# JADGardner/neusky

Hardware: AMD Instinct MI355X
Metric: train rays/sec on NeRF-OSR lk2 @1024 rays x 96 samples (higher is better)
Workload: dtype f32 in memory; forward products: fp16 hi + residual split, 3 x v_mfma_f32_32x32x16_f16 per product on power-of-two pre-scaled operands, one fp32 accumulator (~2^-22): FiLM-SIREN chains and the SDF / albedo field alike; backward products: the same fp16 split on per-row / per-matrix pre-scaled gradien; 1 GPU; full NeuSky train step (BASELINE configs[2]): 1024 rays/GPU x 96 samples, proposal 256+96, 512 illumination directions (256 upper-hemisphere DDF queries/ray), illumination decoder = this project's FiLM-SIREN H = 128 (RENI-shaped: latent 100x3; the reference's configured Attention decoder is absent from its tree), hash L16 F2 T2^19 x2, 256-wide MLPs; fwd + losses + bwd + all-reduce + 5 Adam groups; rays_per_gpu=1024, samples_per_ray=96, illumination_directions=512, parallelism=ray-sharded dp1, launcher=self-spawned, launch=HIP graph replay (1 graph/step + all-reduce + 5 Adam launches)

## Files before the change

neusky_amd/csrc/film_chain.hip:

```cpp
#include "chain.h"

namespace {

constexpr int FWD_FRAG_BUFFERS = 3;


struct Layout {
  int NT, Gc, Gx, Gh;
  long base_map, base_film0, base_film, base_head, total_groups;
  int n_tiles;
};

__host__ __device__ inline Layout fwd_layout(const nsky_film_net& n) {
  Layout L;
  L.NT = n.hidden / 32;
  L.Gc = groups_of(n.cond_dim);
  L.Gx = groups_of(n.x_dim);
  L.Gh = groups_of(n.hidden);
  L.base_map = (long)L.NT * L.Gc;
  L.base_film0 = L.base_map + (long)(n.n_map - 1) * L.NT * L.Gh;
  L.base_film = L.base_film0 + (long)L.NT * (2 * L.Gh + L.Gx);
  L.base_head = L.base_film + (long)(n.n_film - 1) * L.NT * 3 * L.Gh;
  L.total_groups = L.base_head + L.Gh;
  L.n_tiles = n.n_map * L.NT + n.n_film * L.NT * 3 + 1;
// ... 128 lines not shown

struct FwdArgs {
  nsky_film_net net;
  const unsigned char* stream;
  const float* table;
  const float* cond; int ldcond;
  const float* x; int ldx;
  int M;
  float* h_save[MAXL];
  float* z_save[MAXL];
  float* y_save[MAXL];
  float* res; int ldres;
};


template <int H, int KSC>
__global__ __launch_bounds__(256, 1) void film_fwd_kernel(const FwdArgs a) {
  constexpr int NT = H / 32, KS = H / 16;
  __shared__ __attribute__((aligned(16))) unsigned char smem[RING_BYTES + (BIAS_FLOATS + SCALE_FLOATS) * 4];
  float* bl = reinterpret_cast<float*>(smem + RING_BYTES);
  const nsky_film_net& net = a.net;
  const int tid = threadIdx.x, lane = tid & 63;
  const int wave = __builtin_amdgcn_readfirstlane(tid >> 6);
  const int c = lane & 31, h = lane >> 5;
  float* sl = bl + BIAS_FLOATS;
  {
    constexpr int N4 = (BIAS_FLOATS + SCALE_FLOATS) / 4;
    float4 q[(N4 + 255) / 256];
#pragma unroll
    for (int i = 0; i < (N4 + 255) / 256; ++i)
      if (i * 256 + tid < N4) q[i] = ldg4(a.table + 4 * (i * 256 + tid));
// ... 94 lines not shown
  }
  f16x8 xh[1], xl[1];
  const float x_inv = load_planes<1>(a.x + rowc * a.ldx, (net.x_dim + 3) & ~3, 1, h, xh, xl);
  f16x8 yh[KS], yl[KS];
#pragma unroll
  for (int ks = 0; ks < KS; ++ks)
#pragma unroll
    for (int j = 0; j < 8; ++j) { yh[ks][j] = (_Float16)0.0f; yl[ks][j] = (_Float16)0.0f; }
  const float* bias_mo = bl + n_map * H;
  const float* bias_film = bias_mo + 2 * n_film * H;
  for (int i = 0; i < n_film; ++i) {
    const float* bF = bias_mo + i * H;
    const float* bP = bias_mo + (n_film + i) * H;
    const float* bZ = bias_film + i * H;
    float* zblk = a.z_save[i] ? a.z_save[i] + (wave_live ? rt : 0) * NT * 1024 : nullptr;
    float* yblk = a.y_save[i] + (wave_live ? rt : 0) * NT * 1024;
    for (int t = 0; t < NT; ++t) {
      f32x16 aF, aP, aZ;
#pragma unroll
      for (int r = 0; r < 16; ++r) { aF[r] = 0.0f; aP[r] = 0.0f; aZ[r] = 0.0f; }
      product<KS, 4, false, RING_GROUPS, FWD_FRAG_BUFFERS>(ws, hh, hl, aF);
      product<KS, 4, false, RING_GROUPS, FWD_FRAG_BUFFERS>(ws, hh, hl, aP);
      float z_unscale;
      if (i == 0) {
        product<1>(ws, xh, xl, aZ);
        z_unscale = x_inv;
      } else {
        product<KS, 4, false, RING_GROUPS, FWD_FRAG_BUFFERS>(ws, yh, yl, aZ);
        z_unscale = 1.0f / Y_SCALE;
      }
      const float iF = h_inv * sl[tile], iP = h_inv * sl[tile + 1], iZ = z_unscale * sl[tile + 2];
// ... 4 lines not shown
        const int fo = 32 * t + 8 * g + 4 * h;
        const float4 b4F = *reinterpret_cast<const float4*>(bF + fo);
        const float4 b4P = *reinterpret_cast<const float4*>(bP + fo);
        const float4 b4Z = *reinterpret_cast<const float4*>(bZ + fo);
        const float bf[4] = {b4F.x, b4F.y, b4F.z, b4F.w}, bp[4] = {b4P.x, b4P.y, b4P.z, b4P.w}, bz[4] = {b4Z.x, b4Z.y, b4Z.z, b4Z.w};
#pragma unroll
        for (int q = 0; q < 4; ++q) {
          const int r = 4 * g + q;
          const float F = fmaf(aF[r], iF, bf[q]), P = fmaf(aP[r], iP, bp[q]), z = fmaf(aZ[r], iZ, bz[q]);
          zz[r] = z;
          yy[r] = sin_cw(fmaf(fmaf(15.0f, F, 30.0f), z, P));
        }
      }
      if (wave_live) {
        if (zblk) store_tile_nt(zblk + t * 1024, lane, zz);
        store_tile(yblk + t * 1024, lane, yy);
      }
    }
#pragma unroll
    for (int ks = 0; ks < KS; ++ks) {
      float x8[8];
#pragma unroll
      for (int u = 0; u < 2; ++u) {
        const float4 q = ldg4_nt(yblk + (ks >> 1) * 1024 + (2 * (ks & 1) + u) * 256 + lane * 4);
        x8[4 * u] = q.x * Y_SCALE; x8[4 * u + 1] = q.y * Y_SCALE; x8[4 * u + 2] = q.z * Y_SCALE; x8[4 * u + 3] = q.w * Y_SCALE;
      }
      split8(x8, yh[ks], yl[ks]);
    }
  }

  {
    f32x16 acc;
// ... 48 lines not shown
}

template <int KSN, int PWN, bool ACTIVE>
__device__ __forceinline__ void prodw(WStream& ws, const f16x8 (&bh)[KSN], const f16x8 (&bl)[KSN], f32x16& acc) {
#pragma unroll
  for (int r = 0; r < 16; ++r) acc[r] = 0.0f;
  if (ACTIVE) product<KSN, PWN>(ws, bh, bl, acc);
  else product_skip<KSN, PWN, false>(ws);
}

template <int OFF>
__device__ __forceinline__ void hidden_load4_s(f32x4& q, const float* sbase, int voff) {
  asm volatile("global_load_dwordx4 %0, %1, %2 offset:%3" : "+v"(q) : "v"(voff), "s"(sbase), "n"(OFF) : "memory");
}

template <int H, bool ACTIVE>
__device__ __forceinline__ void film_bwd4_tile(const BwdFilmArgs& a, WStream& ws, const float* bl, const float* sl, const float* wo, long rt, int lane) {
  constexpr int NT = H / 32, KS = H / 16, GH = (KS + GSLABS - 1) / GSLABS, PW = 4;
  const nsky_film_net& net = a.net;
  const int c = lane & 31, h = lane >> 5;
  const long row = rt * 32 + c;
  const bool live = ACTIVE && row < a.M;
  const long rowc = row < a.M ? row : a.M - 1;
  const int n_film = net.n_film;
  f32x16 dY[NT];
  float h_inv = 1.0f, h_scale = 1.0f;
  if (ACTIVE) {
    float m = 0.0f;
    for (int t = 0; t < NT; ++t) {
      float hv[16];
      load_tile(a.h_last + (rt * NT + t) * 1024, lane, hv);
// ... 35 lines not shown
#pragma unroll
      for (int u = 0; u < 2; ++u) {
        float x8[8];
#pragma unroll
        for (int j = 0; j < 8; ++j) x8[j] = hv[8 * u + j] * h_scale;
        split8(x8, hh[2 * t + u], hl[2 * t + u]);
      }
    }
    asm volatile("s_waitcnt vmcnt(0)" ::: "memory");
  };
  if (ACTIVE && H_RESIDENT) load_h();
  for (int i = n_film - 1; i >= 0; --i) {
    const float* bF = bias_mo + i * H;
    const float* bP = bias_mo + (n_film + i) * H;
    const float* zp = a.z_save[i] + rt * NT * 1024;
    float* dzp = a.dz_save[i] + rt * NT * 1024;
    float* dFp = a.dfp + (rt * (2 * n_film * NT) + (long)i * NT) * 1024;
    float* dPp = a.dfp + (rt * (2 * n_film * NT) + (long)(n_film + i) * NT) * 1024;
    float dz_max = 0.0f;
    {
      if (ACTIVE && !H_RESIDENT) load_h();
#pragma unroll
      for (int t = 0; t < NT; ++t) {
        f32x4 zq[4];
        int toff = t * 1024;
        asm volatile("" : "+s"(toff));
        const float* zpt = zp + toff;
        float *dzt = dzp + toff, *dFt = dFp + toff, *dPt = dPp + toff;
        if (ACTIVE) {
#pragma unroll
          for (int g = 0; g < 4; ++g) zq[g] = f32x4{0.f, 0.f, 0.f, 0.f};
// ... 16 lines not shown
            const float bf[4] = {b4F.x, b4F.y, b4F.z, b4F.w}, bp[4] = {b4P.x, b4P.y, b4P.z, b4P.w};
            float dzv[4], dFv[4], dPv[4];
#pragma unroll
            for (int q = 0; q < 4; ++q) {
              const int r = 4 * g + q;
              const float F = fmaf(aF[r], iF, bf[q]), P = fmaf(aP[r], iP, bp[q]), z = zq[g][q];
              const float f = fmaf(15.0f, F, 30.0f);
              const float gc = dY[t][r] * cos_cw(fmaf(f, z, P));
              dzv[q] = gc * f;
              dFv[q] = 15.0f * gc * z;
              dPv[q] = gc;
              dY[t][r] = dzv[q];
              dz_max = fmaxf(dz_max, fabsf(dzv[q]));
              fp_max = fmaxf(fp_max, fmaxf(fabsf(dFv[q]), fabsf(gc)));
            }
            stg4(dzt + (g * 256 + lane * 4), make_float4(dzv[0], dzv[1], dzv[2], dzv[3]));
            stg4(dFt + (g * 256 + lane * 4), make_float4(dFv[0], dFv[1], dFv[2], dFv[3]));
            stg4(dPt + (g * 256 + lane * 4), make_float4(dPv[0], dPv[1], dPv[2], dPv[3]));
            asm volatile("" : "+v"(dz_max), "+v"(fp_max));
          }
        }
        tile += 2;
      }
    }
    {
      float dz_inv = 1.0f;
      f16x8 dh_[KS], dl_[KS];
      if (ACTIVE) {
        publish_max(a.gmax + i, dz_max, live, true, lane);
        const float s = row_scale(dz_max, dz_inv);
#pragma unroll
        for (int ks = 0; ks < KS; ++ks) {
          float x8[8];
#pragma unroll
          for (int j = 0; j < 8; ++j) x8[j] = dY[ks >> 1][8 * (ks & 1) + j] * s;
          split8(x8, dh_[ks], dl_[ks]);
        }
      }
      if (i > 0) {
#pragma unroll
        for (int u = 0; u < NT; ++u) {
          f32x16 acc;
          prodw<KS, PW, ACTIVE>(ws, dh_, dl_, acc);
          if (ACTIVE) {
// ... 12 lines not shown
          for (int g = 0; g < 2; ++g)
            if (8 * g + 4 * h < a.ldx)
              stg4(a.d_x + row * a.ldx + 8 * g + 4 * h, make_float4(acc[4 * g] * inv, acc[4 * g + 1] * inv, acc[4 * g + 2] * inv, acc[4 * g + 3] * inv));
        }
        ++tile;
      }
    }
  }
  if (ACTIVE) {
    fp_max = fmaxf(fp_max, __shfl_xor(fp_max, 32, 64));
    if (h == 0) a.dfp_rowmax[row] = fp_max;
    publish_max(a.gmax + n_film, fp_max, live, true, lane);
  }
}

template <int H>
__global__ __launch_bounds__(256, 1) void film_bwd4_kernel(const BwdFilmArgs a) {
  __shared__ __attribute__((aligned(16))) unsigned char smem[RING_BYTES + (BIAS_FLOATS + SCALE_FLOATS) * 4 + 4 * H * 4];
  float* bl = reinterpret_cast<float*>(smem + RING_BYTES);
  float* sl = bl + BIAS_FLOATS;
  float* wo = sl + SCALE_FLOATS;
  const nsky_film_net& net = a.net;
  const int tid = threadIdx.x, lane = tid & 63;
  const int wave = __builtin_amdgcn_readfirstlane(tid >> 6);
  {
    constexpr int N4 = (BIAS_FLOATS + SCALE_FLOATS) / 4;
    float4 q[(N4 + 255) / 256];
#pragma unroll
    for (int i = 0; i < (N4 + 255) / 256; ++i)
      if (i * 256 + tid < N4) q[i] = ldg4(a.table + 4 * (i * 256 + tid));
#pragma unroll
    for (int i = 0; i < (N4 + 255) / 256; ++i)
      if (i * 256 + tid < N4) *reinterpret_cast<float4*>(bl + 4 * (i * 256 + tid)) = q[i];
    for (int i = tid; i < 4 * H; i += 256) wo[i] = (i / H) < net.out_dim ? net.out_w[(long)(i / H) * net.out_ld + (i % H)] : 0.0f;
  }
  __syncthreads();
  asm volatile("s_waitcnt vmcnt(0)" ::: "memory");
  WStream ws;
  ws.src = a.stream + wave * 4096 + lane * 16;
  ws.dst = (uint32_t)(uintptr_t)smem + wave * 4096;
  ws.lds_lane = (uint32_t)(uintptr_t)smem + lane * 16;
  ws_begin(ws);
  const long n_tiles = (a.M + 31) / 32;
  const long rt = (long)blockIdx.x * 4 + wave;
  if (rt < n_tiles) film_bwd4_tile<H, true>(a, ws, bl, sl, wo, rt, lane);
  else film_bwd4_tile<H, false>(a, ws, bl, sl, wo, 0, lane);
  asm volatile("s_waitcnt vmcnt(0) lgkmcnt(0)" ::: "memory");
}

struct BwdMapArgs {
  nsky_film_net net;
  const unsigned char* stream;
  const float* table;
  int M;
  const float* dfp;
  const float* dfp_rowmax;
  const float* h_save[MAXL];
  float* dpre_save[MAXL];
  float* d_cond; int ldcond;
  float* gmax;
  int full_wgs, tail_wgs, tail_k;
};

template <int H, bool ACTIVE>
__device__ __forceinline__ void film_bwd_map_tile(const BwdMapArgs& a, WStream& ws, const float* sl, long rt, int lane) {
  constexpr int NT = H / 32, KS = H / 16, PW = 2;
  const nsky_film_net& net = a.net;
  const int c = lane & 31, h = lane >> 5;
  const long row = rt * 32 + c;
  const bool live = ACTIVE && row < a.M;
  const int nkb = 2 * net.n_film * H / 64, ntot = 2 * net.n_film * NT;
  float f_inv = 1.0f, f_scale = 1.0f;
  if (ACTIVE) f_scale = row_scale(a.dfp_rowmax[rt * 32 + c], f_inv);
  int tile = 0;
  const float* fblk = a.dfp + rt * ntot * 1024;
  const int top = net.n_map - 1;
  float m = 0.0f;
  f32x4 fq[8];
#define NSKY_FQ_WAIT(N)                                                                                                         \
  asm volatile("s_waitcnt vmcnt(%8)"                                                                                            \
               : "+v"(fq[0]), "+v"(fq[1]), "+v"(fq[2]), "+v"(fq[3]), "+v"(fq[4]), "+v"(fq[5]), "+v"(fq[6]), "+v"(fq[7])           \
// ... 48 lines not shown
    }
    if (ACTIVE) NSKY_FQ_WAIT(PW * (NT / 2));
  }
  if (ACTIVE) {
#pragma unroll
    for (int u = 0; u < NT; ++u) {
      const float inv = f_inv * sl[tile - NT + u];
      float hv[16], dv[16];
      load_tile(a.h_save[top] + (rt * NT + u) * 1024, lane, hv);
#pragma unroll
      for (int r = 0; r < 16; ++r) {
        const float g = dh[u][r] * inv;
        dv[r] = hv[r] > 0.0f ? g : 0.2f * g;
        m = fmaxf(m, fabsf(dv[r]));
      }
      store_tile(a.dpre_save[top] + (rt * NT + u) * 1024, lane, dv);
    }
    asm volatile("s_waitcnt vmcnt(0)" ::: "memory");
  }
#undef NSKY_FQ_WAIT

  for (int l = top; l >= 0; --l) {
    float d_inv = 1.0f;
    f16x8 ph[KS], pl[KS];
    if (ACTIVE) {
      publish_max(a.gmax + l, m, live, true, lane);
      const float s = row_scale(m, d_inv);
#pragma unroll
      for (int u = 0; u < NT; ++u) {
        float dv[16];
        load_tile(a.dpre_save[l] + (rt * NT + u) * 1024, lane, dv);
#pragma unroll
        for (int v = 0; v < 2; ++v) {
          float x8[8];
#pragma unroll
          for (int j = 0; j < 8; ++j) x8[j] = dv[8 * v + j] * s;
          split8(x8, ph[2 * u + v], pl[2 * u + v]);
        }
      }
      asm volatile("s_waitcnt vmcnt(0)" ::: "memory");
    }
    m = 0.0f;
    if (l > 0) {
      for (int u = 0; u < NT; ++u) {
        f32x16 acc;
        prodw<KS, PW, ACTIVE>(ws, ph, pl, acc);
        if (ACTIVE) {
          const float inv = d_inv * sl[tile];
          float hv[16], dv[16];
          load_tile(a.h_save[l - 1] + (rt * NT + u) * 1024, lane, hv);
#pragma unroll
          for (int r = 0; r < 16; ++r) {
            const float g = acc[r] * inv;
            dv[r] = hv[r] > 0.0f ? g : 0.2f * g;
            m = fmaxf(m, fabsf(dv[r]));
          }
          store_tile(a.dpre_save[l - 1] + (rt * NT + u) * 1024, lane, dv);
          asm volatile("s_waitcnt vmcnt(0)" ::: "memory");
        }
        ++tile;
      }
    } else {
      const int ct = (net.cond_dim + 31) / 32;
      for (int u = 0; u < ct; ++u) {
        f32x16 acc;
        prodw<KS, PW, ACTIVE>(ws, ph, pl, acc);
        if (ACTIVE && a.d_cond && live) {
          const float inv = d_inv * sl[tile];
#pragma unroll
          for (int g = 0; g < 4; ++g) {
            const int fo = 32 * u + 8 * g + 4 * h;
            if (fo < a.ldcond)
              stg4(a.d_cond + row * a.ldcond + fo, make_float4(acc[4 * g] * inv, acc[4 * g + 1] * inv, acc[4 * g + 2] * inv, acc[4 * g + 3] * inv));
          }
        }
        ++tile;
      }
    }
  }
}

template <int H>
__global__ __launch_bounds__(512, 2) void film_bwd_map_kernel(const BwdMapArgs a) {
  constexpr int PW = 2;
  __shared__ __attribute__((aligned(16))) unsigned char smem[RING_BYTES + SCALE_FLOATS * 4];
  float* sl = reinterpret_cast<float*>(smem + RING_BYTES);
  const int tid = threadIdx.x, lane = tid & 63;
  const int wave = __builtin_amdgcn_readfirstlane(tid >> 6);
  for (int i = tid; i < SCALE_FLOATS; i += 512) sl[i] = a.table[BIAS_FLOATS + i];
  __syncthreads();
  asm volatile("s_waitcnt vmcnt(0)" ::: "memory");
  WStream ws;
  ws.src = a.stream + wave * (PW * 1024) + lane * 16;
  ws.dst = (uint32_t)(uintptr_t)smem + wave * (PW * 1024);
  ws.lds_lane = (uint32_t)(uintptr_t)smem + lane * 16;
  ws_begin<PW>(ws);
  const long n_tiles = (a.M + 31) / 32;
  const long rt = tail_tile(a.full_wgs, a.tail_wgs, a.tail_k, n_tiles, wave);
  if (rt >= 0 && rt < n_tiles) film_bwd_map_tile<H, true>(a, ws, sl, rt, lane);
  else film_bwd_map_tile<H, false>(a, ws, sl, 0, lane);
  asm volatile("s_waitcnt vmcnt(0) lgkmcnt(0)" ::: "memory");
}

struct SdfLayout { int NT, G0, Gh, KS0; };
__host__ __device__ inline SdfLayout sdf_layout(const nsky_sdf_net& n) {
  SdfLayout L;
  L.NT = n.hidden / 32; L.KS0 = ksteps_of(n.in_dim); L.G0 = groups_of(n.in_dim); L.Gh = groups_of(n.hidden);
  return L;
}
__host__ __device__ inline void sdf_dir_layout(const nsky_sdf_net& n, int direction, long& total_groups, int& n_tiles) {
  const SdfLayout L = sdf_layout(n);
  if (direction == 0) { n_tiles = 2 * L.NT; total_groups = (long)L.NT * (L.G0 + L.Gh); }
  else { const int ct = (n.in_dim + 31) / 32; n_tiles = L.NT + ct; total_groups = (long)(L.NT + ct) * L.Gh; }
}
__device__ inline TileDesc sdf_tile(const nsky_sdf_net& n, int direction, int idx) {
// ... 340 lines not shown
  NSKY_CHECK_ARG(direction >= 0 && direction <= 2 && stream_buf && table && ((uintptr_t)stream_buf % 16) == 0 && ((uintptr_t)table % 16) == 0, "nsky_film_pack: bad arguments");
  long groups;
  int tiles;
  dir_layout(*net, direction, groups, tiles);
  NSKY_CHECK_ARG(tiles <= SCALE_FLOATS, "nsky_film_pack: %d weight tiles exceed the scale table (%d)", tiles, SCALE_FLOATS);
  if (direction != 0) NSKY_CHECK_ARG(net->hidden % 128 == 0, "nsky_film_pack: backward streams need hidden %% 128 == 0");
  hipLaunchKernelGGL(film_pack_kernel, dim3(tiles + 1), dim3(256), 0, (hipStream_t)stream, *net, direction, (unsigned char*)stream_buf, table);
  NSKY_CHECK_LAUNCH("nsky_film_pack");
  return NSKY_OK;
}

extern "C" int nsky_film_chain_fwd(const nsky_film_net* net, const void* stream_buf, const float* table, const float* cond,
                                   int32_t ldcond, const float* x, int32_t ldx, int32_t M, float* const* h_save, float* const* z_save,
                                   float* const* y_save, float* res, int32_t ldres, nsky_stream_t stream) {
  if (int rc = check_net(net, "nsky_film_chain_fwd")) return rc;
  NSKY_CHECK_ARG(stream_buf && table && cond && x && res && y_save && M > 0, "nsky_film_chain_fwd: null operand / empty batch");
  NSKY_CHECK_ARG(ldcond % 4 == 0 && ldcond >= ((net->cond_dim + 3) & ~3) && ldx % 4 == 0 && ldx >= ((net->x_dim + 3) & ~3) && ldres >= 4 && ldres % 4 == 0,
                 "nsky_film_chain_fwd: leading dimensions (cond %d, x %d, res %d) must be multiples of 4 covering the padded widths", ldcond, ldx, ldres);
  NSKY_CHECK_ARG(((uintptr_t)cond % 16) == 0 && ((uintptr_t)x % 16) == 0 && ((uintptr_t)res % 16) == 0 && ((uintptr_t)stream_buf % 16) == 0 && ((uintptr_t)table % 16) == 0,
                 "nsky_film_chain_fwd: operands must be 16-byte aligned");
  FwdArgs a;
  a.net = *net;
  a.stream = (const unsigned char*)stream_buf; a.table = table;
  a.cond = cond; a.ldcond = ldcond; a.x = x; a.ldx = ldx; a.M = M; a.res = res; a.ldres = ldres;
  for (int l = 0; l < MAXL; ++l) {
    a.h_save[l] = (h_save && l < net->n_map) ? h_save[l] : nullptr;
    a.z_save[l] = (z_save && l < net->n_film) ? z_save[l] : nullptr;
    a.y_save[l] = l < net->n_film ? y_save[l] : nullptr;
    if (l < net->n_film) NSKY_CHECK_ARG(a.y_save[l] && ((uintptr_t)a.y_save[l] % 16) == 0, "nsky_film_chain_fwd: y_save[%d] missing / unaligned", l);
  }
  const dim3 grid(ceil_div(M, 128));
  const int ksc = ksteps_of(net->cond_dim);
#define NSKY_FILM_FWD(HH, KK) hipLaunchKernelGGL((film_fwd_kernel<HH, KK>), grid, dim3(256), 0, (hipStream_t)stream, a)
  if (net->hidden == 256) { if (ksc <= 4) NSKY_FILM_FWD(256, 4); else NSKY_FILM_FWD(256, 20); }
  else { if (ksc <= 4) NSKY_FILM_FWD(128, 4); else NSKY_FILM_FWD(128, 20); }
#undef NSKY_FILM_FWD
  NSKY_CHECK_LAUNCH("nsky_film_chain_fwd");
  return NSKY_OK;
}


extern "C" int nsky_film_chain_bwd_film(const nsky_film_net* net, const void* stream_buf, const float* table, int32_t M, const float* d_res,
                                        int32_t ldres, const float* h_last, const float* const* z_save, float* const* dz_save, float* dfp,
                                        float* dfp_rowmax, float* gmax, float* d_x, int32_t ldx, nsky_stream_t stream) {
  if (int rc = check_net(net, "nsky_film_chain_bwd_film")) return rc;
  NSKY_CHECK_ARG(stream_buf && table && d_res && h_last && z_save && dz_save && dfp && dfp_rowmax && gmax && M > 0, "nsky_film_chain_bwd_film: null operand / empty batch");
  NSKY_CHECK_ARG(ldres >= 4 && ldres % 4 == 0 && ((uintptr_t)d_res % 16) == 0 && ((uintptr_t)h_last % 16) == 0 && ((uintptr_t)dfp % 16) == 0 &&
                     ((uintptr_t)stream_buf % 16) == 0 && ((uintptr_t)table % 16) == 0, "nsky_film_chain_bwd_film: alignment / ldres");
  NSKY_CHECK_ARG(net->hidden % 128 == 0, "nsky_film_chain_bwd_film: hidden %% 128");
  BwdFilmArgs a;
  a.net = *net; a.stream = (const unsigned char*)stream_buf; a.table = table; a.M = M; a.d_res = d_res; a.ldres = ldres; a.h_last = h_last;
  a.dfp = dfp; a.dfp_rowmax = dfp_rowmax; a.gmax = gmax; a.d_x = d_x; a.ldx = ldx;
  if (d_x) NSKY_CHECK_ARG(ldx % 4 == 0 && ldx >= ((net->x_dim + 3) & ~3) && ldx <= 16 && ((uintptr_t)d_x % 16) == 0, "nsky_film_chain_bwd_film: d_x layout (ldx %d)", ldx);
  for (int l = 0; l < MAXL; ++l) {
    a.z_save[l] = l < net->n_film ? z_save[l] : nullptr;
    a.dz_save[l] = l < net->n_film ? dz_save[l] : nullptr;
    if (l < net->n_film) NSKY_CHECK_ARG(a.z_save[l] && a.dz_save[l] && ((uintptr_t)a.z_save[l] % 16) == 0 && ((uintptr_t)a.dz_save[l] % 16) == 0, "nsky_film_chain_bwd_film: z_save / dz_save[%d]", l);
  }
  a.full_wgs = a.tail_wgs = a.tail_k = 0;
  const dim3 grid(ceil_div(ceil_div(M, 32), 4));
  if (net->hidden == 256) hipLaunchKernelGGL((film_bwd4_kernel<256>), grid, dim3(256), 0, (hipStream_t)stream, a);
  else hipLaunchKernelGGL((film_bwd4_kernel<128>), grid, dim3(256), 0, (hipStream_t)stream, a);
  NSKY_CHECK_LAUNCH("nsky_film_chain_bwd_film");
  return NSKY_OK;
}

extern "C" int nsky_film_chain_bwd_map(const nsky_film_net* net, const void* stream_buf, const float* table, int32_t M, const float* dfp,
                                       const float* dfp_rowmax, const float* const* h_save, float* const* dpre_save, float* d_cond,
                                       int32_t ldcond, float* gmax, nsky_stream_t stream) {
  if (int rc = check_net(net, "nsky_film_chain_bwd_map")) return rc;
  NSKY_CHECK_ARG(stream_buf && table && dfp && dfp_rowmax && h_save && dpre_save && gmax && M > 0, "nsky_film_chain_bwd_map: null operand / empty batch");
  NSKY_CHECK_ARG(((uintptr_t)dfp % 16) == 0 && ((uintptr_t)stream_buf % 16) == 0 && ((uintptr_t)table % 16) == 0, "nsky_film_chain_bwd_map: alignment");
  if (d_cond) NSKY_CHECK_ARG(ldcond % 4 == 0 && ldcond >= ((net->cond_dim + 3) & ~3) && ((uintptr_t)d_cond % 16) == 0, "nsky_film_chain_bwd_map: d_cond layout");
  NSKY_CHECK_ARG(net->hidden % 128 == 0, "nsky_film_chain_bwd_map: hidden %% 128");
  BwdMapArgs a;
  a.net = *net; a.stream = (const unsigned char*)stream_buf; a.table = table; a.M = M; a.dfp = dfp; a.dfp_rowmax = dfp_rowmax;
  a.d_cond = d_cond; a.ldcond = ldcond; a.gmax = gmax;
  for (int l = 0; l < MAXL; ++l) {
    a.h_save[l] = l < net->n_map ? h_save[l] : nullptr;
    a.dpre_save[l] = l < net->n_map ? dpre_save[l] : nullptr;
    if (l < net->n_map) NSKY_CHECK_ARG(a.h_save[l] && a.dpre_save[l] && ((uintptr_t)a.h_save[l] % 16) == 0 && ((uintptr_t)a.dpre_save[l] % 16) == 0, "nsky_film_chain_bwd_map: h_save / dpre_save[%d]", l);
  }
  const TailPlan tp = tail_plan(ceil_div(M, 32), device_cus());
  a.full_wgs = tp.full_wgs; a.tail_wgs = tp.tail_wgs; a.tail_k = tp.tail_k;
  const dim3 grid(tp.full_wgs + tp.tail_wgs);
  if (net->hidden == 256) hipLaunchKernelGGL((film_bwd_map_kernel<256>), grid, dim3(512), 0, (hipStream_t)stream, a);
  else hipLaunchKernelGGL((film_bwd_map_kernel<128>), grid, dim3(512), 0, (hipStream_t)stream, a);
  NSKY_CHECK_LAUNCH("nsky_film_chain_bwd_map");
  return NSKY_OK;
}

extern "C" int nsky_sdf_stream_layout(const nsky_sdf_net* net, int32_t direction, int64_t* stream_bytes, int32_t* n_tiles) {
  if (int rc = check_sdf_net(net, "nsky_sdf_stream_layout")) return rc;
  NSKY_CHECK_ARG(direction == 0 || direction == 1, "nsky_sdf_stream_layout: direction %d", direction);
  long groups; int tiles;
  sdf_dir_layout(*net, direction, groups, tiles);
  if (stream_bytes) *stream_bytes = (groups + RING_GROUPS + 2) * (int64_t)GROUP;
  if (n_tiles) *n_tiles = tiles;
  return NSKY_OK;
}

extern "C" int nsky_sdf_pack(const nsky_sdf_net* net, int32_t direction, void* stream_buf, float* table, nsky_stream_t stream) {
// ... 51 lines not shown
```

neusky_amd/hip.py:

```python
from __future__ import annotations

import ctypes as C
import os

import torch

_HERE = os.path.dirname(os.path.abspath(__file__))
LIB_PATH = os.path.join(_HERE, "libneusky_hip.so")


class NeuSkyHipError(RuntimeError):
    pass


if not os.path.exists(LIB_PATH):
    raise ImportError(
        f"{LIB_PATH} not found: build the HIP extension first (python -c 'import __graft_entry__ as g; g.build()'). "
        "neusky_amd has no CPU/PyTorch fallback."
    )
_lib = C.CDLL(LIB_PATH)

EPI_NONE, EPI_RELU, EPI_LEAKY, EPI_SIGMOID, EPI_SOFTPLUS, EPI_FILM, EPI_MUL_AUX = 0, 1, 2, 3, 4, 5, 6
EPI_BWD_RELU, EPI_BWD_LEAKY, EPI_BWD_FILM, EPI_EXP = 7, 8, 9, 10
PREC_F32, PREC_BF16X2, PREC_BF16X3, PREC_F16X2 = 0, 2, 3, 4
# ... 947 lines not shown
    check(_native_wcolsum(ptr(X), nt, rows, ptr(w4), n_out, ptr(g_sdf), ptr(g_grad), ptr(out), ld(out) if out.dim() == 2 else out.shape[0],
                          ptr(bias), stream_ptr()), "nsky_native_weighted_colsum")


def quad_native_to_rows(buf, N: int, width: int):
    return film_native_to_rows(buf, 4 * N, width).reshape(N, 4, width).permute(1, 0, 2)


def _ptr_array(ts, n):
    arr = (C.c_void_p * FILM_MAX_LAYERS)()
    for i in range(n):
        arr[i] = None if ts is None or ts[i] is None else ts[i].data_ptr()
    return arr


def film_chain_fwd(net: FilmNet, stream_buf, scales, cond, x, M, h_save, z_save, y_save, res):
    check(_film_fwd(C.byref(net), ptr(stream_buf), ptr(scales), ptr(cond), ld(cond), ptr(x), ld(x), M,
                    _ptr_array(h_save, net.n_map), _ptr_array(z_save, net.n_film), _ptr_array(y_save, net.n_film), ptr(res), ld(res),
                    stream_ptr()), "nsky_film_chain_fwd")
    return res


def film_rows(M: int) -> int:
    return (M + 31) // 32 * 32


def film_native_to_rows(buf, M: int, width: int):
    R = film_rows(M) // 32
    return buf.reshape(R, width // 32, 4, 2, 32, 4).permute(0, 4, 1, 2, 3, 5).reshape(R * 32, width)[:M]

# ... 213 lines not shown
```

neusky_amd/ops.py:

```python
from __future__ import annotations

from typing import List, Optional, Sequence

import torch
import torch.nn.functional as F

from . import hip


_POLICIES = ("f32", "splith")
_FWD = {"splith": hip.PREC_F16X2}
_POLICY = "splith"
FWD_PRECISION = _FWD.get(_POLICY, hip.PREC_F32)
BWD_PRECISION = hip.PREC_F32


def set_precision_policy(policy: str) -> None:
    global FWD_PRECISION, _POLICY
    if policy not in _POLICIES:
        raise ValueError(policy)
    _POLICY = policy
    FWD_PRECISION = _FWD.get(policy, hip.PREC_F32)


# ... 598 lines not shown
        stream, table = _stream_buffers(("film", stable_id(wb[0]), n_map, n_film, direction), nbytes, hip.FILM_TABLE_FLOATS, wb[0].device)
        hip.film_pack(net, stream, table, direction)
        return net, stream, table
    return _prepared(_FILM_STREAMS, key, list(wb), pack)


class FilmChainFn(torch.autograd.Function):

    @staticmethod
    def forward(ctx, x, cond, n_map, n_film, train_weights, need_dcond, *wb):
        M = x.shape[0]
        dev = x.device
        mw, _, _, _, fw, _, ow, _, _ = _film_unpack(wb, n_map, n_film)
        H, Hm, n_out_p = fw[0].shape[0], mw[0].shape[0], ow.shape[0]
        save = any(ctx.needs_input_grad)
        net, stream, scales = _film_stream(wb, n_map, n_film)
        Mp = hip.film_rows(M)
        ys = [torch.empty(Mp, H, device=dev) for _ in range(n_film if save else min(2, n_film))]
        hs = [torch.empty(Mp, Hm, device=dev) for _ in range(n_map)] if save else None
        zs = [torch.empty(Mp, H, device=dev) for _ in range(n_film)] if save else None
        res = torch.empty(M, n_out_p, device=dev)
        hip.film_chain_fwd(net, stream, scales, cond, x, M, hs, zs, ys if save else [ys[i % len(ys)] for i in range(n_film)], res)
        if not save:
            return res
        ctx.save_for_backward(x, cond, *hs, *ys, *zs, *wb)
        ctx.cfg = (n_map, n_film, train_weights, need_dcond, M, H, Hm, x.requires_grad)
        ctx.sinks = [_sink_param(w) for w in wb]
        ctx.pad_sinks = [_sink_param(w, "pad") for w in wb]
        return res

    @staticmethod
    def backward(ctx, d_res):
        n_map, n_film, train_w, need_dcond, M, H, Hm, need_dx = ctx.cfg
        train_w = train_w and any(ctx.needs_input_grad[6:])
        sv = ctx.saved_tensors
        x, cond = sv[0], sv[1]
        hs = list(sv[2:2 + n_map])
        ys = list(sv[2 + n_map:2 + n_map + n_film])
        zs = list(sv[2 + n_map + n_film:2 + n_map + 2 * n_film])
        wb = sv[2 + n_map + 2 * n_film:]
        mw, mb, mwo, mbo, fw, fb, ow, ob, o = _film_unpack(wb, n_map, n_film)
        dev = x.device
        Mp = hip.film_rows(M)
        d_res = d_res.contiguous()
        net1, s1, t1 = _film_stream(wb, n_map, n_film, 1)
        net2, s2, t2 = _film_stream(wb, n_map, n_film, 2)
        dzs = [torch.empty(Mp, H, device=dev) for _ in range(n_film)]
        dfp = torch.empty(Mp, 2 * n_film * H, device=dev)
        rowmax = torch.empty(Mp, device=dev)
        gmax = zeros(n_film + 1 + n_map, device=dev)
        d_x = torch.empty(M, ld(x), device=dev) if need_dx else None
        hip.film_chain_bwd_film(net1, s1, t1, M, d_res, hs[-1], zs, dzs, dfp, rowmax, gmax[:n_film + 1], d_x)
        d_cond = torch.empty(M, ld(cond), device=dev) if need_dcond else None
        want_map = need_dcond or train_w
        dpres = [torch.empty(Mp, Hm, device=dev) for _ in range(n_map)] if want_map else None
        if want_map:
            hip.film_chain_bwd_map(net2, s2, t2, M, dfp, rowmax, hs, dpres, d_cond, gmax[n_film + 1:])
        if not train_w:
            return (d_x, d_cond, None, None, None, None, *[None] * len(wb))
        grads, sunk = _carve_grads(wb, _sink_grads(ctx.sinks, from_first_pass=True))
        nt, ntm = H // 32, Hm // 32
        native = []

        def wgrad(dZ, X, n_out, k_in, like, bias_like, iw, a_nt, b_nt, smax, x_scale=64.0):
            if a_nt > 0 and b_nt > 0 and a_nt % 4 == 0 and b_nt % 4 == 0 and smax is not None:
                native.append(hip.wgrad_problem(dZ, a_nt, X, b_nt, M, grads[iw], grads[iw + 1], smax, x_scale))
            elif a_nt == 0 and b_nt > 0 and n_out <= 4 and dZ.dim() == 2 and dZ.shape[1] == 4 and dZ.is_contiguous():
                hip.native_weighted_colsum(X, b_nt, M, grads[iw], grads[iw + 1], w4=dZ, n_out=n_out)
            else:
                grad_weight(dZ, X, M, n_out, k_in, like, bias_like, acc=(grads[iw], grads[iw + 1]), a_native_nt=a_nt, b_native_nt=b_nt,
# ... 1122 lines not shown
```

Before: 52670 rays/s.

## Skip saving FiLM chain activations and gradients when weights are not trained

```diff
diff --git a/neusky_amd/csrc/film_chain.hip b/neusky_amd/csrc/film_chain.hip
--- a/neusky_amd/csrc/film_chain.hip
+++ b/neusky_amd/csrc/film_chain.hip
@@ -166,7 +166,7 @@
 };
 
 
-template <int H, int KSC>
+template <int H, int KSC, bool KEEP_Y = true>
 __global__ __launch_bounds__(256, 1) void film_fwd_kernel(const FwdArgs a) {
   constexpr int NT = H / 32, KS = H / 16;
   __shared__ __attribute__((aligned(16))) unsigned char smem[RING_BYTES + (BIAS_FLOATS + SCALE_FLOATS) * 4];
@@ -291,7 +291,8 @@
     const float* bP = bias_mo + (n_film + i) * H;
     const float* bZ = bias_film + i * H;
     float* zblk = a.z_save[i] ? a.z_save[i] + (wave_live ? rt : 0) * NT * 1024 : nullptr;
-    float* yblk = a.y_save[i] + (wave_live ? rt : 0) * NT * 1024;
+    float* yblk = KEEP_Y ? a.y_save[i] + (wave_live ? rt : 0) * NT * 1024 : nullptr;
+    f16x8 nh[KEEP_Y ? 1 : KS], nl[KEEP_Y ? 1 : KS];
     for (int t = 0; t < NT; ++t) {
       f32x16 aF, aP, aZ;
 #pragma unroll
@@ -326,8 +327,26 @@
       }
       if (wave_live) {
         if (zblk) store_tile_nt(zblk + t * 1024, lane, zz);
-        store_tile(yblk + t * 1024, lane, yy);
-      }
+        if constexpr (KEEP_Y) store_tile(yblk + t * 1024, lane, yy);
+      }
+      if constexpr (!KEEP_Y) {
+#pragma unroll
+        for (int tt = 0; tt < NT; ++tt)
+          if (t == tt) {
+#pragma unroll
+            for (int u = 0; u < 2; ++u) {
+              float x8[8];
+#pragma unroll
+              for (int j = 0; j < 8; ++j) x8[j] = yy[8 * u + j] * Y_SCALE;
+              split8(x8, nh[2 * tt + u], nl[2 * tt + u]);
+            }
+          }
+      }
+    }
+    if constexpr (!KEEP_Y) {
+#pragma unroll
+      for (int ks = 0; ks < KS; ++ks) { yh[ks] = nh[ks]; yl[ks] = nl[ks]; }
+      continue;
     }
 #pragma unroll
     for (int ks = 0; ks < KS; ++ks) {
@@ -406,7 +425,7 @@
   asm volatile("global_load_dwordx4 %0, %1, %2 offset:%3" : "+v"(q) : "v"(voff), "s"(sbase), "n"(OFF) : "memory");
 }
 
-template <int H, bool ACTIVE>
+template <int H, bool ACTIVE, bool KEEP>
 __device__ __forceinline__ void film_bwd4_tile(const BwdFilmArgs& a, WStream& ws, const float* bl, const float* sl, const float* wo, long rt, int lane) {
   constexpr int NT = H / 32, KS = H / 16, GH = (KS + GSLABS - 1) / GSLABS, PW = 4;
   const nsky_film_net& net = a.net;
@@ -472,7 +491,7 @@
     const float* bF = bias_mo + i * H;
     const float* bP = bias_mo + (n_film + i) * H;
     const float* zp = a.z_save[i] + rt * NT * 1024;
-    float* dzp = a.dz_save[i] + rt * NT * 1024;
+    float* dzp = KEEP ? a.dz_save[i] + rt * NT * 1024 : nullptr;
     float* dFp = a.dfp + (rt * (2 * n_film * NT) + (long)i * NT) * 1024;
     float* dPp = a.dfp + (rt * (2 * n_film * NT) + (long)(n_film + i) * NT) * 1024;
     float dz_max = 0.0f;
@@ -519,9 +538,14 @@
               dz_max = fmaxf(dz_max, fabsf(dzv[q]));
               fp_max = fmaxf(fp_max, fmaxf(fabsf(dFv[q]), fabsf(gc)));
             }
-            stg4(dzt + (g * 256 + lane * 4), make_float4(dzv[0], dzv[1], dzv[2], dzv[3]));
-            stg4(dFt + (g * 256 + lane * 4), make_float4(dFv[0], dFv[1], dFv[2], dFv[3]));
-            stg4(dPt + (g * 256 + lane * 4), make_float4(dPv[0], dPv[1], dPv[2], dPv[3]));
+            if constexpr (KEEP) {
+              stg4(dzt + (g * 256 + lane * 4), make_float4(dzv[0], dzv[1], dzv[2], dzv[3]));
+              stg4(dFt + (g * 256 + lane * 4), make_float4(dFv[0], dFv[1], dFv[2], dFv[3]));
+              stg4(dPt + (g * 256 + lane * 4), make_float4(dPv[0], dPv[1], dPv[2], dPv[3]));
+            } else {
+              *reinterpret_cast<f32x4*>(dFt + (g * 256 + lane * 4)) = f32x4{dFv[0], dFv[1], dFv[2], dFv[3]};
+              *reinterpret_cast<f32x4*>(dPt + (g * 256 + lane * 4)) = f32x4{dPv[0], dPv[1], dPv[2], dPv[3]};
+            }
             asm volatile("" : "+v"(dz_max), "+v"(fp_max));
           }
         }
@@ -532,7 +556,7 @@
       float dz_inv = 1.0f;
       f16x8 dh_[KS], dl_[KS];
       if (ACTIVE) {
-        publish_max(a.gmax + i, dz_max, live, true, lane);
+        if constexpr (KEEP) publish_max(a.gmax + i, dz_max, live, true, lane);
         const float s = row_scale(dz_max, dz_inv);
 #pragma unroll
         for (int ks = 0; ks < KS; ++ks) {
@@ -575,7 +599,7 @@
   }
 }
 
-template <int H>
+template <int H, bool KEEP = true>
 __global__ __launch_bounds__(256, 1) void film_bwd4_kernel(const BwdFilmArgs a) {
   __shared__ __attribute__((aligned(16))) unsigned char smem[RING_BYTES + (BIAS_FLOATS + SCALE_FLOATS) * 4 + 4 * H * 4];
   float* bl = reinterpret_cast<float*>(smem + RING_BYTES);
@@ -604,8 +628,8 @@
   ws_begin(ws);
   const long n_tiles = (a.M + 31) / 32;
   const long rt = (long)blockIdx.x * 4 + wave;
-  if (rt < n_tiles) film_bwd4_tile<H, true>(a, ws, bl, sl, wo, rt, lane);
-  else film_bwd4_tile<H, false>(a, ws, bl, sl, wo, 0, lane);
+  if (rt < n_tiles) film_bwd4_tile<H, true, KEEP>(a, ws, bl, sl, wo, rt, lane);
+  else film_bwd4_tile<H, false, KEEP>(a, ws, bl, sl, wo, 0, lane);
   asm volatile("s_waitcnt vmcnt(0) lgkmcnt(0)" ::: "memory");
 }
 
@@ -623,9 +647,11 @@
   int full_wgs, tail_wgs, tail_k;
 };
 
-template <int H, bool ACTIVE>
+template <int H, bool ACTIVE, bool KEEP>
 __device__ __forceinline__ void film_bwd_map_tile(const BwdMapArgs& a, WStream& ws, const float* sl, long rt, int lane) {
   constexpr int NT = H / 32, KS = H / 16, PW = 2;
+  constexpr bool REGS = !KEEP && H <= 128;
+  float dreg[REGS ? NT : 1][16];
   const nsky_film_net& net = a.net;
   const int c = lane & 31, h = lane >> 5;
   const long row = rt * 32 + c;
@@ -704,7 +730,12 @@
         dv[r] = hv[r] > 0.0f ? g : 0.2f * g;
         m = fmaxf(m, fabsf(dv[r]));
       }
-      store_tile(a.dpre_save[top] + (rt * NT + u) * 1024, lane, dv);
+      if constexpr (REGS) {
+#pragma unroll
+        for (int r = 0; r < 16; ++r) dreg[u][r] = dv[r];
+      } else {
+        store_tile(a.dpre_save[top] + (rt * NT + u) * 1024, lane, dv);
+      }
     }
     asm volatile("s_waitcnt vmcnt(0)" ::: "memory");
   }
@@ -714,12 +745,17 @@
     float d_inv = 1.0f;
     f16x8 ph[KS], pl[KS];
     if (ACTIVE) {
-      publish_max(a.gmax + l, m, live, true, lane);
+      if constexpr (KEEP) publish_max(a.gmax + l, m, live, true, lane);
       const float s = row_scale(m, d_inv);
 #pragma unroll
       for (int u = 0; u < NT; ++u) {
         float dv[16];
-        load_tile(a.dpre_save[l] + (rt * NT + u) * 1024, lane, dv);
+        if constexpr (REGS) {
+#pragma unroll
+          for (int r = 0; r < 16; ++r) dv[r] = dreg[u][r];
+        } else {
+          load_tile(a.dpre_save[l] + (rt * NT + u) * 1024, lane, dv);
+        }
 #pragma unroll
         for (int v = 0; v < 2; ++v) {
           float x8[8];
@@ -745,7 +781,16 @@
             dv[r] = hv[r] > 0.0f ? g : 0.2f * g;
             m = fmaxf(m, fabsf(dv[r]));
           }
-          store_tile(a.dpre_save[l - 1] + (rt * NT + u) * 1024, lane, dv);
+          if constexpr (REGS) {
+#pragma unroll
+            for (int uu = 0; uu < NT; ++uu)
+              if (u == uu) {
+#pragma unroll
+                for (int r = 0; r < 16; ++r) dreg[uu][r] = dv[r];
+              }
+          } else {
+            store_tile(a.dpre_save[l - 1] + (rt * NT + u) * 1024, lane, dv);
+          }
           asm volatile("s_waitcnt vmcnt(0)" ::: "memory");
         }
         ++tile;
@@ -770,7 +815,7 @@
   }
 }
 
-template <int H>
+template <int H, bool KEEP = true>
 __global__ __launch_bounds__(512, 2) void film_bwd_map_kernel(const BwdMapArgs a) {
   constexpr int PW = 2;
   __shared__ __attribute__((aligned(16))) unsigned char smem[RING_BYTES + SCALE_FLOATS * 4];
@@ -787,8 +832,8 @@
   ws_begin<PW>(ws);
   const long n_tiles = (a.M + 31) / 32;
   const long rt = tail_tile(a.full_wgs, a.tail_wgs, a.tail_k, n_tiles, wave);
-  if (rt >= 0 && rt < n_tiles) film_bwd_map_tile<H, true>(a, ws, sl, rt, lane);
-  else film_bwd_map_tile<H, false>(a, ws, sl, 0, lane);
+  if (rt >= 0 && rt < n_tiles) film_bwd_map_tile<H, true, KEEP>(a, ws, sl, rt, lane);
+  else film_bwd_map_tile<H, false, KEEP>(a, ws, sl, 0, lane);
   asm volatile("s_waitcnt vmcnt(0) lgkmcnt(0)" ::: "memory");
 }
 
@@ -1159,7 +1204,7 @@
                                    int32_t ldcond, const float* x, int32_t ldx, int32_t M, float* const* h_save, float* const* z_save,
                                    float* const* y_save, float* res, int32_t ldres, nsky_stream_t stream) {
   if (int rc = check_net(net, "nsky_film_chain_fwd")) return rc;
-  NSKY_CHECK_ARG(stream_buf && table && cond && x && res && y_save && M > 0, "nsky_film_chain_fwd: null operand / empty batch");
+  NSKY_CHECK_ARG(stream_buf && table && cond && x && res && M > 0, "nsky_film_chain_fwd: null operand / empty batch");
   NSKY_CHECK_ARG(ldcond % 4 == 0 && ldcond >= ((net->cond_dim + 3) & ~3) && ldx % 4 == 0 && ldx >= ((net->x_dim + 3) & ~3) && ldres >= 4 && ldres % 4 == 0,
                  "nsky_film_chain_fwd: leading dimensions (cond %d, x %d, res %d) must be multiples of 4 covering the padded widths", ldcond, ldx, ldres);
   NSKY_CHECK_ARG(((uintptr_t)cond % 16) == 0 && ((uintptr_t)x % 16) == 0 && ((uintptr_t)res % 16) == 0 && ((uintptr_t)stream_buf % 16) == 0 && ((uintptr_t)table % 16) == 0,
@@ -1171,14 +1216,18 @@
   for (int l = 0; l < MAXL; ++l) {
     a.h_save[l] = (h_save && l < net->n_map) ? h_save[l] : nullptr;
     a.z_save[l] = (z_save && l < net->n_film) ? z_save[l] : nullptr;
-    a.y_save[l] = l < net->n_film ? y_save[l] : nullptr;
-    if (l < net->n_film) NSKY_CHECK_ARG(a.y_save[l] && ((uintptr_t)a.y_save[l] % 16) == 0, "nsky_film_chain_fwd: y_save[%d] missing / unaligned", l);
-  }
+    a.y_save[l] = (y_save && l < net->n_film) ? y_save[l] : nullptr;
+  }
+  const bool keep_y = a.y_save[0] != nullptr;
+  NSKY_CHECK_ARG(keep_y || net->hidden == 128, "nsky_film_chain_fwd: NULL y_save needs hidden 128 (hidden %d: pass two ping-pong buffers)", net->hidden);
+  for (int l = 0; l < net->n_film; ++l)
+    NSKY_CHECK_ARG((a.y_save[l] != nullptr) == keep_y && ((uintptr_t)a.y_save[l] % 16) == 0, "nsky_film_chain_fwd: y_save[%d] missing / unaligned", l);
   const dim3 grid(ceil_div(M, 128));
   const int ksc = ksteps_of(net->cond_dim);
-#define NSKY_FILM_FWD(HH, KK) hipLaunchKernelGGL((film_fwd_kernel<HH, KK>), grid, dim3(256), 0, (hipStream_t)stream, a)
-  if (net->hidden == 256) { if (ksc <= 4) NSKY_FILM_FWD(256, 4); else NSKY_FILM_FWD(256, 20); }
-  else { if (ksc <= 4) NSKY_FILM_FWD(128, 4); else NSKY_FILM_FWD(128, 20); }
+#define NSKY_FILM_FWD(HH, KK, KEEP) hipLaunchKernelGGL((film_fwd_kernel<HH, KK, KEEP>), grid, dim3(256), 0, (hipStream_t)stream, a)
+  if (net->hidden == 256) { if (ksc <= 4) NSKY_FILM_FWD(256, 4, true); else NSKY_FILM_FWD(256, 20, true); }
+  else if (keep_y) { if (ksc <= 4) NSKY_FILM_FWD(128, 4, true); else NSKY_FILM_FWD(128, 20, true); }
+  else { if (ksc <= 4) NSKY_FILM_FWD(128, 4, false); else NSKY_FILM_FWD(128, 20, false); }
 #undef NSKY_FILM_FWD
   NSKY_CHECK_LAUNCH("nsky_film_chain_fwd");
   return NSKY_OK;
@@ -1189,7 +1238,7 @@
                                         int32_t ldres, const float* h_last, const float* const* z_save, float* const* dz_save, float* dfp,
                                         float* dfp_rowmax, float* gmax, float* d_x, int32_t ldx, nsky_stream_t stream) {
   if (int rc = check_net(net, "nsky_film_chain_bwd_film")) return rc;
-  NSKY_CHECK_ARG(stream_buf && table && d_res && h_last && z_save && dz_save && dfp && dfp_rowmax && gmax && M > 0, "nsky_film_chain_bwd_film: null operand / empty batch");
+  NSKY_CHECK_ARG(stream_buf && table && d_res && h_last && z_save && dfp && dfp_rowmax && gmax && M > 0, "nsky_film_chain_bwd_film: null operand / empty batch");
   NSKY_CHECK_ARG(ldres >= 4 && ldres % 4 == 0 && ((uintptr_t)d_res % 16) == 0 && ((uintptr_t)h_last % 16) == 0 && ((uintptr_t)dfp % 16) == 0 &&
                      ((uintptr_t)stream_buf % 16) == 0 && ((uintptr_t)table % 16) == 0, "nsky_film_chain_bwd_film: alignment / ldres");
   NSKY_CHECK_ARG(net->hidden % 128 == 0, "nsky_film_chain_bwd_film: hidden %% 128");
@@ -1199,13 +1248,17 @@
   if (d_x) NSKY_CHECK_ARG(ldx % 4 == 0 && ldx >= ((net->x_dim + 3) & ~3) && ldx <= 16 && ((uintptr_t)d_x % 16) == 0, "nsky_film_chain_bwd_film: d_x layout (ldx %d)", ldx);
   for (int l = 0; l < MAXL; ++l) {
     a.z_save[l] = l < net->n_film ? z_save[l] : nullptr;
-    a.dz_save[l] = l < net->n_film ? dz_save[l] : nullptr;
-    if (l < net->n_film) NSKY_CHECK_ARG(a.z_save[l] && a.dz_save[l] && ((uintptr_t)a.z_save[l] % 16) == 0 && ((uintptr_t)a.dz_save[l] % 16) == 0, "nsky_film_chain_bwd_film: z_save / dz_save[%d]", l);
-  }
+    a.dz_save[l] = (dz_save && l < net->n_film) ? dz_save[l] : nullptr;
+  }
+  const bool keep = a.dz_save[0] != nullptr;
+  for (int l = 0; l < net->n_film; ++l)
+    NSKY_CHECK_ARG(a.z_save[l] && (a.dz_save[l] != nullptr) == keep && ((uintptr_t)a.z_save[l] % 16) == 0 && ((uintptr_t)a.dz_save[l] % 16) == 0, "nsky_film_chain_bwd_film: z_save / dz_save[%d]", l);
   a.full_wgs = a.tail_wgs = a.tail_k = 0;
   const dim3 grid(ceil_div(ceil_div(M, 32), 4));
-  if (net->hidden == 256) hipLaunchKernelGGL((film_bwd4_kernel<256>), grid, dim3(256), 0, (hipStream_t)stream, a);
-  else hipLaunchKernelGGL((film_bwd4_kernel<128>), grid, dim3(256), 0, (hipStream_t)stream, a);
+#define NSKY_FILM_BWD4(HH, KEEP) hipLaunchKernelGGL((film_bwd4_kernel<HH, KEEP>), grid, dim3(256), 0, (hipStream_t)stream, a)
+  if (net->hidden == 256) { if (keep) NSKY_FILM_BWD4(256, true); else NSKY_FILM_BWD4(256, false); }
+  else { if (keep) NSKY_FILM_BWD4(128, true); else NSKY_FILM_BWD4(128, false); }
+#undef NSKY_FILM_BWD4
   NSKY_CHECK_LAUNCH("nsky_film_chain_bwd_film");
   return NSKY_OK;
 }
@@ -1214,7 +1267,7 @@
                                        const float* dfp_rowmax, const float* const* h_save, float* const* dpre_save, float* d_cond,
                                        int32_t ldcond, float* gmax, nsky_stream_t stream) {
   if (int rc = check_net(net, "nsky_film_chain_bwd_map")) return rc;
-  NSKY_CHECK_ARG(stream_buf && table && dfp && dfp_rowmax && h_save && dpre_save && gmax && M > 0, "nsky_film_chain_bwd_map: null operand / empty batch");
+  NSKY_CHECK_ARG(stream_buf && table && dfp && dfp_rowmax && h_save && gmax && M > 0, "nsky_film_chain_bwd_map: null operand / empty batch");
   NSKY_CHECK_ARG(((uintptr_t)dfp % 16) == 0 && ((uintptr_t)stream_buf % 16) == 0 && ((uintptr_t)table % 16) == 0, "nsky_film_chain_bwd_map: alignment");
   if (d_cond) NSKY_CHECK_ARG(ldcond % 4 == 0 && ldcond >= ((net->cond_dim + 3) & ~3) && ((uintptr_t)d_cond % 16) == 0, "nsky_film_chain_bwd_map: d_cond layout");
   NSKY_CHECK_ARG(net->hidden % 128 == 0, "nsky_film_chain_bwd_map: hidden %% 128");
@@ -1223,14 +1276,21 @@
   a.d_cond = d_cond; a.ldcond = ldcond; a.gmax = gmax;
   for (int l = 0; l < MAXL; ++l) {
     a.h_save[l] = l < net->n_map ? h_save[l] : nullptr;
-    a.dpre_save[l] = l < net->n_map ? dpre_save[l] : nullptr;
-    if (l < net->n_map) NSKY_CHECK_ARG(a.h_save[l] && a.dpre_save[l] && ((uintptr_t)a.h_save[l] % 16) == 0 && ((uintptr_t)a.dpre_save[l] % 16) == 0, "nsky_film_chain_bwd_map: h_save / dpre_save[%d]", l);
-  }
+    a.dpre_save[l] = (dpre_save && l < net->n_map) ? dpre_save[l] : nullptr;
+  }
+  const bool regs = a.dpre_save[0] == nullptr;
+  const bool keep = !regs && !(net->n_map > 1 && a.dpre_save[1] == a.dpre_save[0]);
+  NSKY_CHECK_ARG(!regs || net->hidden == 128, "nsky_film_chain_bwd_map: NULL dpre_save needs hidden 128 (hidden %d: pass one shared buffer)", net->hidden);
+  for (int l = 0; l < net->n_map; ++l)
+    NSKY_CHECK_ARG(a.h_save[l] && (a.dpre_save[l] == nullptr) == regs && (keep || a.dpre_save[l] == a.dpre_save[0]) && ((uintptr_t)a.h_save[l] % 16) == 0 &&
+                       ((uintptr_t)a.dpre_save[l] % 16) == 0, "nsky_film_chain_bwd_map: h_save / dpre_save[%d]", l);
   const TailPlan tp = tail_plan(ceil_div(M, 32), device_cus());
   a.full_wgs = tp.full_wgs; a.tail_wgs = tp.tail_wgs; a.tail_k = tp.tail_k;
   const dim3 grid(tp.full_wgs + tp.tail_wgs);
-  if (net->hidden == 256) hipLaunchKernelGGL((film_bwd_map_kernel<256>), grid, dim3(512), 0, (hipStream_t)stream, a);
-  else hipLaunchKernelGGL((film_bwd_map_kernel<128>), grid, dim3(512), 0, (hipStream_t)stream, a);
+#define NSKY_FILM_BWD_MAP(HH, KEEP) hipLaunchKernelGGL((film_bwd_map_kernel<HH, KEEP>), grid, dim3(512), 0, (hipStream_t)stream, a)
+  if (net->hidden == 256) { if (keep) NSKY_FILM_BWD_MAP(256, true); else NSKY_FILM_BWD_MAP(256, false); }
+  else { if (keep) NSKY_FILM_BWD_MAP(128, true); else NSKY_FILM_BWD_MAP(128, false); }
+#undef NSKY_FILM_BWD_MAP
   NSKY_CHECK_LAUNCH("nsky_film_chain_bwd_map");
   return NSKY_OK;
 }
diff --git a/neusky_amd/hip.py b/neusky_amd/hip.py
--- a/neusky_amd/hip.py
+++ b/neusky_amd/hip.py
@@ -985,6 +985,10 @@
     return arr
 
 
+def film_keepless(hidden: int) -> str:
+    return "registers" if hidden == 128 else "buffers"
+
+
 def film_chain_fwd(net: FilmNet, stream_buf, scales, cond, x, M, h_save, z_save, y_save, res):
     check(_film_fwd(C.byref(net), ptr(stream_buf), ptr(scales), ptr(cond), ld(cond), ptr(x), ld(x), M,
                     _ptr_array(h_save, net.n_map), _ptr_array(z_save, net.n_film), _ptr_array(y_save, net.n_film), ptr(res), ld(res),
diff --git a/neusky_amd/ops.py b/neusky_amd/ops.py
--- a/neusky_amd/ops.py
+++ b/neusky_amd/ops.py
@@ -636,17 +636,25 @@
         mw, _, _, _, fw, _, ow, _, _ = _film_unpack(wb, n_map, n_film)
         H, Hm, n_out_p = fw[0].shape[0], mw[0].shape[0], ow.shape[0]
         save = any(ctx.needs_input_grad)
+        train_w = train_weights and any(ctx.needs_input_grad[6:])
+        keep_y = save and train_w
         net, stream, scales = _film_stream(wb, n_map, n_film)
         Mp = hip.film_rows(M)
-        ys = [torch.empty(Mp, H, device=dev) for _ in range(n_film if save else min(2, n_film))]
+        if keep_y:
+            ys = [torch.empty(Mp, H, device=dev) for _ in range(n_film)]
+        elif save and hip.film_keepless(H) == "registers":
+            ys = None
+        else:
+            pp = [torch.empty(Mp, H, device=dev) for _ in range(min(2, n_film))]
+            ys = [pp[i % len(pp)] for i in range(n_film)]
         hs = [torch.empty(Mp, Hm, device=dev) for _ in range(n_map)] if save else None
         zs = [torch.empty(Mp, H, device=dev) for _ in range(n_film)] if save else None
         res = torch.empty(M, n_out_p, device=dev)
-        hip.film_chain_fwd(net, stream, scales, cond, x, M, hs, zs, ys if save else [ys[i % len(ys)] for i in range(n_film)], res)
+        hip.film_chain_fwd(net, stream, scales, cond, x, M, hs, zs, ys, res)
         if not save:
             return res
-        ctx.save_for_backward(x, cond, *hs, *ys, *zs, *wb)
-        ctx.cfg = (n_map, n_film, train_weights, need_dcond, M, H, Hm, x.requires_grad)
+        ctx.save_for_backward(x, cond, *hs, *(ys if keep_y else []), *zs, *wb)
+        ctx.cfg = (n_map, n_film, train_w, need_dcond, M, H, Hm, x.requires_grad)
         ctx.sinks = [_sink_param(w) for w in wb]
         ctx.pad_sinks = [_sink_param(w, "pad") for w in wb]
         return res
@@ -654,20 +662,20 @@
     @staticmethod
     def backward(ctx, d_res):
         n_map, n_film, train_w, need_dcond, M, H, Hm, need_dx = ctx.cfg
-        train_w = train_w and any(ctx.needs_input_grad[6:])
         sv = ctx.saved_tensors
         x, cond = sv[0], sv[1]
         hs = list(sv[2:2 + n_map])
-        ys = list(sv[2 + n_map:2 + n_map + n_film])
-        zs = list(sv[2 + n_map + n_film:2 + n_map + 2 * n_film])
-        wb = sv[2 + n_map + 2 * n_film:]
+        n_ys = n_film if train_w else 0
+        ys = list(sv[2 + n_map:2 + n_map + n_ys])
+        zs = list(sv[2 + n_map + n_ys:2 + n_map + n_ys + n_film])
+        wb = sv[2 + n_map + n_ys + n_film:]
         mw, mb, mwo, mbo, fw, fb, ow, ob, o = _film_unpack(wb, n_map, n_film)
         dev = x.device
         Mp = hip.film_rows(M)
         d_res = d_res.contiguous()
         net1, s1, t1 = _film_stream(wb, n_map, n_film, 1)
         net2, s2, t2 = _film_stream(wb, n_map, n_film, 2)
-        dzs = [torch.empty(Mp, H, device=dev) for _ in range(n_film)]
+        dzs = [torch.empty(Mp, H, device=dev) for _ in range(n_film)] if train_w else None
         dfp = torch.empty(Mp, 2 * n_film * H, device=dev)
         rowmax = torch.empty(Mp, device=dev)
         gmax = zeros(n_film + 1 + n_map, device=dev)
@@ -675,7 +683,12 @@
         hip.film_chain_bwd_film(net1, s1, t1, M, d_res, hs[-1], zs, dzs, dfp, rowmax, gmax[:n_film + 1], d_x)
         d_cond = torch.empty(M, ld(cond), device=dev) if need_dcond else None
         want_map = need_dcond or train_w
-        dpres = [torch.empty(Mp, Hm, device=dev) for _ in range(n_map)] if want_map else None
+        if train_w:
+            dpres = [torch.empty(Mp, Hm, device=dev) for _ in range(n_map)]
+        elif want_map and hip.film_keepless(Hm) == "buffers":
+            dpres = [torch.empty(Mp, Hm, device=dev)] * n_map
+        else:
+            dpres = None
         if want_map:
             hip.film_chain_bwd_map(net2, s2, t2, M, dfp, rowmax, hs, dpres, d_cond, gmax[n_film + 1:])
         if not train_w:
```

After: 54340 rays/s, median of 6. 1.03x the previous value.
